# gvtulder/elasticdeform

Measured on AMD Instinct MI355X. Metric: Mvoxels/s fwd+grad, 256^3 fp32 order=3, higher is better.
Workload: dtype f32; 1 GPU; cfg2: 3D 256x256x256 float32, 5x5x5 grid sigma 5, order 3, mode mirror, prefilter on, deform_grid + deform_grid_gradient per step, one volume per GPU; parallelism=1 volume per GPU, no collective

## Files before the change

### elasticdeform_amd/csrc/deform_k1z.hip

```cpp
#include <hip/hip_runtime.h>

#include <cstring>
#include <type_traits>

#include "ed_device.h"
#include "ed_gridfilter.h"
#include "ed_params.h"
#include "ed_tile.h"
#include "ed_workspace.h"
#include "ed_zwalk.h"

namespace ed {
namespace tile {

#ifdef EDHIP_K1_STATS
__device__ unsigned long long g_k1z_stats[8];
#define ZSTAT(K, N) atomicAdd(&g_k1z_stats[K], (unsigned long long)(N))
#else
#define ZSTAT(K, N) do { } while (0)
#endif

namespace {


enum : int {
    kZAny = 1,
    kZStaged = 2,
    kZFast = 4,
    kZDma = 8,
    kZXin = 16,
    kZZYin = 32,
    kZUnfit = 64,
    kZGen = 128,
};
struct ZRecU {
    int b0z, b0y, b0x, flags, pitch, ez, ey, ex, goff, plane;
};
typedef int zv8i __attribute__((ext_vector_type(8)));
typedef const __attribute__((address_space(4))) zv8i* crec_p;
__device__ __forceinline__ ZRecU zrec_unpack(const zv8i& v)
{
    ZRecU r;
    r.b0z = v[0];
    r.b0y = v[1];
    r.b0x = v[2];
    r.flags = v[3];
    r.pitch = (v[3] >> 8) & 255;
    r.ez = v[4] & 1023;
    r.ey = (v[4] >> 10) & 1023;
    r.ex = (int)((unsigned)v[4] >> 20);
    r.goff = v[5];
    r.plane = r.ey * r.pitch;
    return r;
}
__device__ __forceinline__ ZRecU zrec_load(crec_p p)
{
    const zv8i v = *p;
    return zrec_unpack(v);
}

enum : int { kZHeavy = 0, kZFix = 1, kZLight = 2, kZCursor = 3 };
__host__ __device__ __forceinline__ int zctl(int parity, int word, int xcd) { return (parity * 4 + word) * 8 + xcd; }

__device__ __forceinline__ void zaxis_entry(const GridGeom& g, int a, int oi, double* w, int* idx)
{
    const double cp = control_coordinate(g.ncp[a], (int64_t)oi + g.off[a], g.in_len[a]);
    const int64_t start = window_start(cp, 3);
    const bool edge = start < 0 || start + 3 >= g.ncp[a];
    spline_weights(cp, 3, w);
#pragma unroll
    for (int l = 0; l < 4; ++l)
        idx[l] = edge ? mirror_i32((int)start + l, (int)g.ncp[a]) : (int)start + l;
}

constexpr int kGeoBlock = 256;
constexpr int kGeoWaves = kGeoBlock / 64;
__global__ __launch_bounds__(kGeoBlock) void k1z_geo_kernel(const GridGeom g, const HotGeom hg, const ZGeom zg,
                                                          const GridPrefilter gp)
{
    extern __shared__ __attribute__((aligned(16))) char smem[];
    const int tid = threadIdx.x;
    const int lane = tid & 63;
    const int wave = uni(tid >> 6);
    const int sample = blockIdx.y;
    const int ncpz = (int)g.ncp[0], ncpy = (int)g.ncp[1], ncpx = (int)g.ncp[2];
    const int nyx = ncpy * ncpx;
    const int ngrid = 3 * ncpz * nyx;
    double* sG = reinterpret_cast<double*>(smem);
    double* sR = sG + ngrid;
    AxTab* sAx = reinterpret_cast<AxTab*>(sR + 64 * ncpz * 3);
    double* sMax = reinterpret_cast<double*>(sAx + 16);
    AxTab* sZ = reinterpret_cast<AxTab*>(sMax + 3 * kGeoWaves);
    int* sCls = reinterpret_cast<int*>(sZ + 4 * hg.tiles[0]);
    int* sBox = sCls + hg.tiles[0];
    int* sCnt = sBox + 64 * hg.tiles[0];
    const int ty = blockIdx.x / hg.tiles[2], tx = blockIdx.x - ty * hg.tiles[2];
    if (ED_DBG(hg.dbg, 1 << 23))
        return;
#ifdef EDHIP_EXPERIMENTS
#define ZTICK(K) do { if (hg.dbgbuf && tid == 0) hg.dbgbuf[(size_t)(blockIdx.x + blockIdx.y * gridDim.x) * 16 + (K)] = __builtin_readcyclecounter(); } while (0)
#else
#define ZTICK(K) do { } while (0)
#endif
    ZTICK(0);

    if (gp.total > 0 && !ED_DBG(hg.dbg, 1 << 28)) {
        grid_prefilter_in_lds<kGeoBlock>(gp, sG, tid);
        if (blockIdx.x == 0 && sample == 0)
            for (int e = tid; e < gp.total; e += kGeoBlock)
                store_cast(gp.out + (int64_t)e * gp.elem_size, gp.dtype, sG[e]);
    } else {
        const char* disp = g.disp + (int64_t)sample * zg.disp_bstride;
        for (int e = tid; e < ngrid; e += kGeoBlock) {
            const int h = e / (ncpz * nyx), r = e - h * (ncpz * nyx);
            const int j0 = r / nyx, j = r - j0 * nyx;
            const int j1 = j / ncpx, j2 = j - j1 * ncpx;
            sG[e] = load_as_double(disp + g.disp_stride[0] * h + g.disp_stride[1] * j0 + g.disp_stride[2] * j1 +
                                       g.disp_stride[3] * j2, g.disp_dtype);
        }
        __syncthreads();
    }
    ZTICK(1);
    if (blockIdx.x == 0 && sample == 0 && tid == 0 && zg.hint) {
        if (zg.hint_host)
            __hip_atomic_store(zg.hint_host, ((unsigned long long)(unsigned)zg.hint[1] << 32) | (unsigned)zg.hint[0],
                               __ATOMIC_RELAXED, __HIP_MEMORY_SCOPE_SYSTEM);
        zg.hint[0] = 0;
        zg.hint[1] = (int)zg.hint_seq;
    }
    for (int h = 0; h < 3 && !ED_DBG(hg.dbg, 1 << 29); ++h) {
        double m = 0.0;
        for (int e = tid; e < ncpz * nyx; e += kGeoBlock)
            m = fmax(m, fabs(sG[h * ncpz * nyx + e]));
        for (int sh = 32; sh >= 1; sh >>= 1)
            m = fmax(m, __shfl_xor(m, sh));
        if (lane == 0)
            sMax[h * kGeoWaves + wave] = m;
    }
    ZTICK(2);
    if (tid < 16 && !ED_DBG(hg.dbg, 1 << 30)) {
        const int a = tid < 8 ? 1 : 2;
        const int oi = min((tid < 8 ? ty : tx) * kT + (tid & 7), hg.out_len[a] - 1);
        AxTab t;
        zaxis_entry(g, a, oi, t.w, t.idx);
        sAx[tid] = t;
    }
    for (int e = tid; e < 4 * hg.tiles[0] && !ED_DBG(hg.dbg, 1 << 26); e += kGeoBlock) {
        const int tz = e >> 2, nz = min(kT, hg.out_len[0] - tz * kT);
        AxTab t;
        zaxis_entry(g, 0, tz * kT + ((e & 3) * (nz - 1)) / 3, t.w, t.idx);
        sZ[e] = t;
    }
    if (blockIdx.x == 0 && sample == 0 && hg.nstep) {
        for (long long ss = tid; ss < hg.nsteps; ss += kGeoBlock) {
            long long vol_off = 0, img_off = 0, r = ss;
            for (int l = 0; l < hg.nstep; ++l) {
                const long long q = r / hg.step_len[l];
                const long long c = r - q * hg.step_len[l];
                vol_off += hg.vol_step[l] * c;
                img_off += hg.img_step[l] * c;
                r = q;
            }
            zg.steps[2 * ss] = vol_off;
            zg.steps[2 * ss + 1] = img_off;
        }
    }
    if (blockIdx.x == 0 && sample == 0 && tid == 0) {
        ZGen* zn = reinterpret_cast<ZGen*>(zg.zgen);
        for (int h = 0; h < 3; ++h) {
            zn->in_len[h] = hg.in_len[h];
            zn->out_len[h] = hg.out_len[h];
            zn->off[h] = hg.off[h];
            zn->period[h] = hg.period[h];
            zn->inv_period[h] = hg.inv_period[h];
            zn->offd[h] = (double)hg.off[h];
        }
        for (int k = 0; k < 12; ++k)
            zn->aff[k] = hg.affine[k];
        zn->mode = hg.mode;
        zn->cval = hg.cval;
        zn->hint = hg.hint;
    }
    if (blockIdx.x == 0 && sample == 0) {
        AxTab* zt = const_cast<AxTab*>(zg.zt);
        for (int oz = tid; oz < hg.out_len[0]; oz += kGeoBlock) {
            AxTab t;
            zaxis_entry(g, 0, oz, t.w, t.idx);
#pragma unroll
            for (int l = 0; l < 4; ++l)
                t.idx[l] *= 32;
            zt[oz] = t;
        }
    }
    __syncthreads();
    ZTICK(3);
    double slack[3];
#pragma unroll
    for (int h = 0; h < 3; ++h) {
        double m = 0.0;
        for (int w = 0; w < kGeoWaves; ++w)
            m = fmax(m, sMax[h * kGeoWaves + w]);
        const double sl = zg.slack_scale * m;
        slack[h] = sl >= 0.02 ? (sl <= 0.75 ? sl : 0.75) : 0.02;
    }
    ZTICK(4);
    if (!ED_DBG(hg.dbg, 1 << 25)) {
        const int col = tid & 63;
        const AxTab ay = sAx[col >> 3];
        const AxTab ax = sAx[8 + (col & 7)];
        int rowoff[4];
#pragma unroll
        for (int ly = 0; ly < 4; ++ly)
            rowoff[ly] = ay.idx[ly] * ncpx;
        for (int r = tid >> 6; r < ncpz * 3; r += kGeoWaves) {
            const int kz = r / 3, h = r - kz * 3;
            const double* gp0 = sG + (h * ncpz + kz) * nyx;
            double acc = 0.0;
#pragma unroll
            for (int ly = 0; ly < 4; ++ly) {
                const double* row = gp0 + rowoff[ly];
                double t = ax.w[0] * row[ax.idx[0]];
#pragma unroll
                for (int lx = 1; lx < 4; ++lx)
                    t = fma(ax.w[lx], row[ax.idx[lx]], t);
                acc = fma(ay.w[ly], t, acc);
            }
            sR[col * (ncpz * 3) + r] = acc;
        }
        __syncthreads();
        double* rg = const_cast<double*>(zg.r) + (int64_t)sample * zg.r_bstride;
        const int rowlen = 8 * 4 * ncpz;
        for (int e = tid; e < 8 * rowlen; e += kGeoBlock) {
            const int py = e / rowlen, j = e - py * rowlen;
            const int px = j / (4 * ncpz), jj = j - px * (4 * ncpz);
            const int kz = jj >> 2, h = jj & 3;
            const int oy = ty * kT + py, ox = tx * kT + px;
            if (oy < hg.out_len[1] && ox < hg.out_len[2])
                rg[((int64_t)oy * hg.out_len[2] + ox) * (4 * ncpz) + jj] = h < 3 ? sR[(py * 8 + px) * (ncpz * 3) + kz * 3 + h] : 0.0;
        }
    }
    __syncthreads();
    ZTICK(5);
    const int order = zg.order;
    const int H = order / 2, NT = order + 1, kPadX = NT & 1;
    const int ny = min(kT, hg.out_len[1] - ty * kT), nx = min(kT, hg.out_len[2] - tx * kT);
    const int py = (((lane >> 2) & 3) * (ny - 1)) / 3, px = ((lane & 3) * (nx - 1)) / 3;
    const double* rc = sR + (py * 8 + px) * (ncpz * 3);
    for (int tz = wave; tz < hg.tiles[0] && !ED_DBG(hg.dbg, 1 << 24); tz += kGeoWaves) {
        const int nz = min(kT, hg.out_len[0] - tz * kT);
        const int pz = ((lane >> 4) * (nz - 1)) / 3;
        const int o[3] = {tz * kT + pz, ty * kT + py, tx * kT + px};
        const AxTab& ze = sZ[tz * 4 + (lane >> 4)];
        double d[3];
#pragma unroll
        for (int h = 0; h < 3; ++h) {
            d[h] = ze.w[0] * rc[ze.idx[0] * 3 + h];
#pragma unroll
            for (int l = 1; l < 4; ++l)
                d[h] = fma(ze.w[l], rc[ze.idx[l] * 3 + h], d[h]);
        }
        double c[3];
        int lo[3], hi[3];
#pragma unroll
        for (int h = 0; h < 3; ++h) {
            if (hg.has_affine)
                c[h] = fma(hg.affine[h * 4 + 2], (double)o[2],
                           fma(hg.affine[h * 4 + 0], (double)o[0],
                               fma(hg.affine[h * 4 + 1], (double)o[1], hg.affine[h * 4 + 3] + (double)hg.off[h]))) + d[h];
            else
                c[h] = (double)(o[h] + hg.off[h]) + d[h];
            const double cr = (order & 1) ? c[h] : c[h] + 0.5;
            lo[h] = (int)floor(cr - slack[h]);
            hi[h] = (int)floor(cr + slack[h]);
        }
        bool out_of_fast = false;
#pragma unroll
        for (int h = 0; h < 3; ++h)
            out_of_fast = out_of_fast || lo[h] < ((order & 1) ? 0 : 1) || hi[h] > hg.in_len[h] - 2;
        const bool fast = nz == kT && ny == kT && nx == kT && !__any(out_of_fast);
        box_reduce<4>(lo, hi);
        int* dst = sBox + (tz * 8 + (lane >> 4)) * 8;
        if ((lane & 15) == 0) {
#pragma unroll
            for (int h = 0; h < 3; ++h) {
                dst[h] = lo[h];
                dst[4 + h] = hi[h];
            }
        }
        if (lane == 0)
            dst[3] = fast ? 1 : 0;
        if (!fast) {
            bool cst = false;
#pragma unroll
            for (int h = 0; h < 3; ++h) {
                double m = c[h];
                if (!(m >= 0.0 && m <= (double)(hg.in_len[h] - 1)))
                    m = map_coordinate_fast(m, hg.in_len[h], hg.mode, hg.period[h], hg.inv_period[h]);
                cst = cst || !(m > -1.0);
                const double mr = (order & 1) ? m : m + 0.5;
                lo[h] = (int)floor(mr - slack[h]);
                hi[h] = (int)floor(mr + slack[h]);
            }
            if (cst) {
#pragma unroll
                for (int h = 0; h < 3; ++h) {
                    lo[h] = 0x7fffffff;
                    hi[h] = (int)0x80000000;
                }
            }
            box_reduce<4>(lo, hi);
            if ((lane & 15) == 0) {
#pragma unroll
                for (int h = 0; h < 3; ++h) {
                    dst[32 + h] = lo[h];
                    dst[36 + h] = hi[h];
                }
            }
        }
    }
    __syncthreads();
    ZTICK(6);
    for (int tz = tid; tz < hg.tiles[0] && !ED_DBG(hg.dbg, 1 << 27); tz += kGeoBlock) {
        const int tile_id = sample * hg.ntiles + (tz * hg.tiles[1] + ty) * hg.tiles[2] + tx;
        int cls = 0;
        bool hint0 = false, slow0 = false, half_fit[2] = {false, false};
#pragma unroll 1
        for (int part = 0; part < 3; ++part) {
            const int* sb = sBox + tz * 64;
            const bool fast = sb[3] != 0;
            const int r0 = part == 2 ? 2 : 0, r1 = part == 1 ? 2 : 3;
            int blo[3], bhi[3];
            bool any = true;
#pragma unroll
            for (int h = 0; h < 3; ++h) {
                int rlo = 0x7fffffff, rhi = (int)0x80000000, lo = 0x7fffffff, hi = (int)0x80000000;
                for (int r = r0; r <= r1; ++r) {
                    rlo = min(rlo, sb[r * 8 + h]);
                    rhi = max(rhi, sb[r * 8 + 4 + h]);
                    lo = min(lo, sb[(fast ? 0 : 32) + r * 8 + h]);
                    hi = max(hi, sb[(fast ? 0 : 32) + r * 8 + 4 + h]);
                }
                if (!fast) {
                    any = any && hi >= lo;
                    const int lowfold = hg.mode == EDHIP_MODE_REFLECT ? -1 : 0;
                    if (rlo < ((order & 1) ? 0 : 1) && rhi >= lowfold)
                        lo = min(lo, lowfold);
                    if (rhi > hg.in_len[h] - 2 && rlo <= hg.in_len[h] - 1)
                        hi = max(hi, hg.in_len[h] - 1);
                }
                blo[h] = lo - H;
                bhi[h] = hi - H + order + (h == 2 ? kPadX : 0);
            }
            if (!any) {
                blo[0] = blo[1] = blo[2] = 0;
                bhi[0] = bhi[1] = bhi[2] = -1;
            }
            any = bhi[0] >= blo[0] && bhi[1] >= blo[1] && bhi[2] >= blo[2];
            unsigned ext[3];
#pragma unroll
            for (int h = 0; h < 3; ++h)
                ext[h] = (unsigned)bhi[h] - (unsigned)blo[h] + 1u;
            const int pitch = ext[2] <= 16u ? 16 : (ext[2] <= 24u ? 24 : (ext[2] <= 32u ? 32 : (ext[2] <= 48u ? 48 : 0)));
            const bool sane = any && ext[0] < 1024u && ext[1] < 1024u;
            const int nrows = sane ? (int)(ext[0] * ext[1]) : 0;
            const bool fits = sane && pitch > 0 && nrows * pitch <= hg.box_cap;
            const bool dma = fits && blo[2] >= 0 && blo[2] + pitch + 1 <= hg.in_len[2];
            const bool xin = fits && blo[2] >= 0 && blo[2] + (int)ext[2] <= hg.in_len[2];
            const bool zyin = fits && blo[0] >= 0 && blo[0] + (int)ext[0] <= hg.in_len[0] && blo[1] >= 0 &&
                              blo[1] + (int)ext[1] <= hg.in_len[1];
            const bool fastA = part == 0 && fast && fits && dma && zyin;
            const int flags = (any ? kZAny : 0) | (fits ? kZStaged : 0) | (fastA ? kZFast : kZGen) | (dma ? kZDma : 0) |
                              (xin ? kZXin : 0) | (zyin ? kZZYin : 0) | (any && !fits ? kZUnfit : 0);
            const int4 w0 = make_int4(blo[0], blo[1], blo[2], flags | (pitch << 8));
            const int4 w1 = make_int4(sane ? (int)(ext[0] | (ext[1] << 10) | (ext[2] << 20)) : 0,
                                      (dma && zyin) ? blo[0] * hg.vol_sz + blo[1] * hg.vol_sy + blo[2] : 0, 0, 0);
            if (part == 0) {
                hint0 = any && !(sane && pitch > 0 && nrows * pitch <= hg.small_cap);
                slow0 = fits && !dma;
                cls = (flags & kZUnfit) ? 3 : ((flags & kZFast) ? 1 : 2);
                int4* dst = reinterpret_cast<int4*>(zg.recs + (size_t)tile_id * 8);
                dst[0] = w0;
                dst[1] = w1;
                if (hg.boxes) {
                    int* bx = hg.boxes + (size_t)tile_id * 8;
#pragma unroll
                    for (int h = 0; h < 3; ++h) {
                        bx[h] = blo[h];
                        bx[3 + h] = bhi[h] - ((h == 2 && any) ? kPadX : 0);
                    }
                }
                if (cls != 3)
                    break;
            } else {
                half_fit[part - 1] = fits || !any;
                int4* dst = reinterpret_cast<int4*>(zg.recs_half + ((size_t)tile_id * 2 + (part - 1)) * 8);
                dst[0] = w0;
                dst[1] = w1;
            }
        }
        const bool split = cls == 3 && half_fit[0] && half_fit[1];
        ZSTAT(cls == 3 ? (split ? 6 : 5) : (cls == 1 ? 3 : 4), 1);
        sCls[tz] = cls | (split ? 4 : 0) | (hint0 ? 8 : 0) | ((cls == 2 && slow0) || split ? 16 : 0);
    }
    __syncthreads();
    ZTICK(7);
    {
        const int zstrips = (hg.tiles[0] + zg.strip_tiles - 1) / zg.strip_tiles;
        int* sCntL = reinterpret_cast<int*>(sMax);
        if (tid < 4)
            sCnt[tid] = 0;
        if (tid < 2)
            sCntL[tid] = 0;
        __syncthreads();
        int slotG = -1, slotL = -1, slotF = -1, sidv = 0;
        if (tid < zstrips) {
            int info = 0, ngen = 0;
            bool slow = false, f = false;
            for (int k = 0; k < zg.strip_tiles && tid * zg.strip_tiles + k < hg.tiles[0]; ++k) {
                const int c = sCls[tid * zg.strip_tiles + k];
                info |= (c & 15) << (4 * k);
                ngen += ((c & 3) == 2 || (c & 7) == 7) ? 1 : 0;
                slow = slow || (c & 16) != 0;
                f = f || (c & 7) == 3;
            }
            const size_t sid = (size_t)sample * zg.nstrips + ((size_t)tid * hg.tiles[1] + ty) * hg.tiles[2] + tx;
            sidv = (int)sid;
            zg.sinfo[sid] = info;
            zg.missed[sid] = f ? 2 : 0;
            if (ngen && (slow || ngen >= 3) && !ED_DBG(hg.dbg, 1 << 13))
                slotG = atomicAdd(&sCnt[0], 1);
            else if (ngen)
                slotL = atomicAdd(&sCntL[0], 1);
            if (f)
                slotF = atomicAdd(&sCnt[1], 1);
        }
        __syncthreads();
        const int xcd = (tx + ty + sample) & 7;
        if (tid == 0) {
            sCnt[2] = sCnt[0] ? atomicAdd(&zg.ctl[zctl(zg.parity, kZHeavy, xcd)], sCnt[0]) : 0;
            sCnt[3] = sCnt[1] ? atomicAdd(&zg.ctl[zctl(zg.parity, kZFix, xcd)], sCnt[1]) : 0;
            sCntL[1] = sCntL[0] ? atomicAdd(&zg.ctl[zctl(zg.parity, kZLight, xcd)], sCntL[0]) : 0;
        }
        if (blockIdx.x == 0 && sample == 0 && tid < 32)
            zg.ctl[zctl(1 - zg.parity, tid >> 3, tid & 7)] = 0;
        __syncthreads();
        if (slotG >= 0)
            zg.list_g[(size_t)(sCnt[2] + slotG) * 8 + xcd] = sidv;
        if (slotL >= 0)
            zg.list_g[(size_t)(zg.total_strips - 1 - (sCntL[1] + slotL)) * 8 + xcd] = sidv;
        if (slotF >= 0)
            zg.list_f[(size_t)(sCnt[3] + slotF) * 8 + xcd] = sidv;
    }
    ZTICK(8);
#undef ZTICK
}


struct ZVox {
    int addr[2];
    float frac[2][3];
    int flg;
};
struct ZStrip {
    int tz0, ty, tx, ntile, sample, id;
};
__device__ __forceinline__ bool k1z_strip(int total_strips, int nstrips, int tiles_z, int tiles_y, int tiles_x, int strip_tiles, int deal,
                                          ZStrip& sp, int b)
{
    const int x = b & 7, j = b >> 3;
    const int r = j / deal;
    int s = (r * 8 + ((x + r) & 7)) * deal + (j - r * deal);
    if (s >= total_strips)
        return false;
    sp.id = s;
    sp.sample = s / nstrips;
    s -= sp.sample * nstrips;
    sp.tx = s % tiles_x;
    s /= tiles_x;
    sp.ty = s % tiles_y;
    sp.tz0 = (s / tiles_y) * strip_tiles;
    sp.ntile = min(strip_tiles, tiles_z - sp.tz0);
    return true;
}
inline unsigned k1z_grid(int total_strips, int deal)
{
    const int chunks = (total_strips + deal - 1) / deal;
    return (unsigned)(((chunks + 7) / 8) * 8 * deal);
}

template <int ORDER, int PITCH>
__device__ __forceinline__ float k1z_gather(const float* bp, int plane, int pitch_rt, const float* w0, const float* w1, const float* w2)
{
    constexpr int NT = ORDER + 1;
    constexpr int NTX = NT + (NT & 1);
    float a0 = 0.f;
#pragma unroll
    for (int l0 = 0; l0 < NT; ++l0) {
        const float* pp = bp + l0 * plane;
        float a1 = 0.f;
#pragma unroll
        for (int l1 = 0; l1 < NT; ++l1) {
            const float* rp = pp + l1 * (PITCH ? PITCH : pitch_rt);
            float a2 = 0.f;
#pragma unroll
            for (int l2 = 0; l2 < NTX; l2 += 2) {
                const float2 pr = *reinterpret_cast<const float2*>(rp + l2);
                ED_NO_DS_MERGE();
                a2 = fmaf(w2[l2], pr.x, a2);
                a2 = fmaf(w2[l2 + 1], pr.y, a2);
            }
            a1 = fmaf(w1[l1], a2, a1);
        }
        a0 = fmaf(w0[l0], a1, a0);
    }
    return a0;
}
template <int ORDER>
__device__ __forceinline__ float k1z_voxel(const char* smem, int addr, const float (&frac)[3], int pitch, int plane)
{
    constexpr int NT = ORDER + 1;
    constexpr int NTX = NT + (NT & 1);
    float f0 = frac[0], f1 = frac[1], f2 = frac[2];
    asm volatile("" : "+v"(f0), "+v"(f1), "+v"(f2));
    float w0[NT], w1[NT], w2[NTX];
    weights_from_frac<float, ORDER>(f0, w0);
    weights_from_frac<float, ORDER>(f1, w1);
    weights_from_frac<float, ORDER>(f2, w2);
    if (NT & 1)
        w2[NT] = 0.f;
    const float* bp = reinterpret_cast<const float*>(smem + addr);
    return pitch == 16 ? k1z_gather<ORDER, 16>(bp, plane, 16, w0, w1, w2) : k1z_gather<ORDER, 0>(bp, plane, pitch, w0, w1, w2);
}

struct ZFast {
    const float* vol;
    float* img;
    const double* r;
    const AxTab* zt;
    const int* recs;
    const int* recs_half;
    int* missed;
    int* hint;
    const int* sinfo;
    const int* list_g;
    int* list_f;
    int* ctl;
    int parity;
    const long long* steps;
    long long vol_bstride, img_bstride, r_bstride;
    int vol_sy, vol_sz, img_sy, img_sz;
    int box_cap, tiles_y, tiles_x, tiles_z, strip_tiles, nstrips, total_strips, ntiles;
    int rcol_bytes, out_y, out_x;
    int kz0, ky0, kx0;
    int io16, nsteps, deal;
    int dbg;
    double aff[12];
#ifdef EDHIP_EXPERIMENTS
    unsigned long long* dbgbuf;
#endif
};
#ifdef EDHIP_EXPERIMENTS
constexpr size_t kZDbgBase = (size_t)1 << 16;
#endif

template <int ORDER, bool AFFINE, bool OUT16, bool STEPS>
__device__ __forceinline__ void k1z_fast_body(const ZFast& a, const int vblock)
{
    constexpr int NT = ORDER + 1;
    constexpr int kPadX = NT & 1;
    constexpr int NTX = NT + kPadX;
    extern __shared__ __attribute__((aligned(16))) char smem[];
    ZStrip sp;
    if (!k1z_strip(a.total_strips, a.nstrips, a.tiles_z, a.tiles_y, a.tiles_x, a.strip_tiles, a.deal, sp, vblock))
        return;
    const int tid = threadIdx.x;
    const int lane = tid & 63;
    const int wave = uni(tid >> 6);
    const int io16 = OUT16 ? a.io16 : 0;
    const int ntile = sp.ntile;
    const size_t tile_step = (size_t)a.tiles_y * a.tiles_x;
    crec_p rec0 = (crec_p)(const void*)a.recs + ((size_t)sp.sample * a.ntiles + ((size_t)sp.tz0 * a.tiles_y + sp.ty) * a.tiles_x + sp.tx);
    const int sinfo = ((cint_p)(const void*)a.sinfo)[sp.id];
    if (a.hint && tid == 0) {
        const int nh = __builtin_popcount((unsigned)sinfo & 0x88888888u);
        if (nh)
            atomicAdd(a.hint, nh);
    }
    auto next_fast = [&](int t) {
        for (++t; t < ntile; ++t)
            if (((sinfo >> (4 * t)) & 3) == 1)
                break;
        return t;
    };
    int ti = next_fast(-1);
    if (ti >= ntile)
        return;

    const int box_cap = a.box_cap;
    const int odd_shift = (box_cap - 1) * 4;
    float* box0 = reinterpret_cast<float*>(smem);
    float* box1 = box0 + box_cap;
    const int vol_sz = a.vol_sz, vol_sy = a.vol_sy, img_sz = a.img_sz;

    const int yy = lane >> 3, xx = lane & 7;
    const int oy = sp.ty * kT + yy, ox = sp.tx * kT + xx;
    const int obase = oy * a.img_sy + ox;
// ... 476 lines not shown
        const int sinfo = ((cint_p)(const void*)a.sinfo)[sp.id];
        const bool missed = (((cint_p)(const void*)a.missed)[sp.id] & 1) != 0;
        if (!STEPS && false)
            (void)steps;
        const int oy = sp.ty * kT + yy, ox = sp.tx * kT + xx;
        const int obase = oy * a.img_sy + ox;
        const float* __restrict__ vol = a.vol + sp.sample * a.vol_bstride;
        float* img = a.img + sp.sample * a.img_bstride;
        const char* rcol = reinterpret_cast<const char*>(a.r + sp.sample * a.r_bstride) +
                           ((size_t)min(oy, a.out_y - 1) * a.out_x + min(ox, a.out_x - 1)) * (size_t)a.rcol_bytes;
        double Pyx[3];
#pragma unroll
        for (int h = 0; h < 3; ++h)
            Pyx[h] = AFFINE ? fma(zn->aff[h * 4 + 2], (double)ox, fma(zn->aff[h * 4 + 1], (double)oy, zn->aff[h * 4 + 3] + zn->offd[h])) : 0.0;
        ZTaps tp;
        tp.key[0] = tp.key[1] = tp.key[2] = tp.key[3] = -1;
        {
            if (missed && lane == 0)
                ZSTAT(0, 1);
            for (int ti = (int)(blockIdx.y >> 1); ti < ntile; ti += ntile) {
                const int c4 = (sinfo >> (4 * ti)) & 7;
                const int cls = c4 & 3;
                const bool split = c4 == 7;
                const bool whole = cls == 3 && !split;
                if (!whole && !missed)
                    continue;
#pragma unroll 1
                for (int i = (int)(blockIdx.y & 1); i < 2; i += 2) {
                    const ZRecU rc = zrec_load(split ? rech0 + ((size_t)ti * tile_step * 2 + i) : rec0 + (size_t)ti * tile_step);
                    const int oz = (sp.tz0 + ti) * kT + wave + 4 * i;
                    if (oz >= zn->out_len[0])
                        continue;
                    double zw[4];
                    k1z_slice(zt, rcol, oz, tp, zw);
                    if (oy >= zn->out_len[1] || ox >= zn->out_len[2])
                        continue;
                    double d[3];
                    k1z_disp(tp, zw, d);
                    const int b[3] = {oz + zn->off[0], oy + zn->off[1], ox + zn->off[2]};
                    double P[3] = {0.0, 0.0, 0.0};
                    if (AFFINE) {
#pragma unroll
                        for (int h = 0; h < 3; ++h)
                            P[h] = fma(zn->aff[h * 4 + 0], (double)oz, Pyx[h]);
                    }
                    int st[3], raw[3];
                    float fr[3];
                    const bool cst = tile_coords<ORDER, AFFINE, float>(zn->in_len, &zn->mode, zn->period, zn->inv_period, d, b,
                                                                       P, st, fr, raw);
                    if (!whole) {
                        const bool gen = cls != 1;
                        if (gen && cst)
                            continue;
                        const int rz = (gen ? st[0] : raw[0]) - rc.b0z, ry = (gen ? st[1] : raw[1]) - rc.b0y,
                                  rx = (gen ? st[2] : raw[2]) - rc.b0x;
                        const bool inside = rz >= 0 && rz + NT <= rc.ez && ry >= 0 && ry + NT <= rc.ey && rx >= 0 &&
                                            rx + NT + kPadX <= rc.ex;
                        if (inside)
                            continue;
                    }
                    int tap[3][NT];
                    float w[3][NT];
#pragma unroll
                    for (int h = 0; h < 3; ++h) {
                        weights_from_frac<float, ORDER>(fr[h], w[h]);
                        const int stride = h == 0 ? vol_sz : (h == 1 ? vol_sy : 1);
#pragma unroll
                        for (int l = 0; l < NT; ++l)
                            tap[h][l] = mirror_i32(st[h] + l, zn->in_len[h]) * stride;
                    }
                    const long long ooff = (long long)oz * img_sz + obase;
                    ZSTAT(whole ? 2 : 1, 1);
                    for (int ss = 0; ss < nsteps; ++ss) {
                        float val = zn->cval;
                        if (!cst) {
                            const float* src = vol + (STEPS ? steps[2 * ss] : 0);
                            float a0 = 0.f;
#pragma unroll
                            for (int l0 = 0; l0 < NT; ++l0) {
                                float a1 = 0.f;
#pragma unroll
                                for (int l1 = 0; l1 < NT; ++l1) {
                                    const float* p1 = src + (tap[0][l0] + tap[1][l1]);
                                    float a2 = 0.f;
#pragma unroll
                                    for (int l2 = 0; l2 < NT; ++l2)
                                        a2 = fmaf(w[2][l2], p1[tap[2][l2]], a2);
                                    a1 = fmaf(w[1][l1], a2, a1);
                                }
                                a0 = fmaf(w[0][l0], a1, a0);
                            }
                            val = a0;
                        }
                        store_out<OUT16>(img, (STEPS ? steps[2 * ss + 1] : 0) + ooff, val, io16);
                    }
                }
            }
        }
    }
}

template <int ORDER, bool AFFINE, bool OUT16, bool STEPS>
hipError_t launch_k1z_kernels(const ZFast& zf, const void* znp, unsigned ngen, unsigned nfix, size_t lds, hipStream_t stream)
{
    const unsigned nfast = k1z_grid(zf.total_strips, zf.deal);
    const unsigned fast_rows = nfast >> 3, gen_rows = ngen >> 3;
    unsigned every = gen_rows ? fast_rows / gen_rows + 1 : 2;
    if (const char* ev = ed_env("EDHIP_ZEVERY"))
        every = (unsigned)atoi(ev);
    if (every < 2)
        every = 2;
    hipLaunchKernelGGL((k1z_tile_kernel<ORDER, AFFINE, OUT16, STEPS>), dim3(nfast + ngen), dim3(kBlock), lds, stream, zf, (czgen_p)znp,
                       (int)ngen, (int)every);
    hipError_t e = hipGetLastError();
    if (e != hipSuccess)
        return e;
    hipLaunchKernelGGL((k1z_fix_kernel<ORDER, AFFINE, OUT16, STEPS>), dim3(nfix, 2 * zf.strip_tiles), dim3(kBlock), 0, stream, zf, (czgen_p)znp);
    return hipGetLastError();
}
template <int ORDER, bool AFFINE, bool OUT16>
hipError_t launch_k1z_variant(const ZFast& zf, const void* zn, unsigned ngen, unsigned nfix, size_t lds, hipStream_t stream,
                              bool steps)
{
    return steps ? launch_k1z_kernels<ORDER, AFFINE, OUT16, true>(zf, zn, ngen, nfix, lds, stream)
                 : launch_k1z_kernels<ORDER, AFFINE, OUT16, false>(zf, zn, ngen, nfix, lds, stream);
}
template <int ORDER>
hipError_t launch_k1z_order(const HotGeom& hg, const ZFast& zf, const void* zn, unsigned ngen, unsigned nfix, size_t lds, hipStream_t stream)
{
    const bool steps = hg.nstep != 0;
    if (hg.io16)
        return hg.has_affine ? launch_k1z_variant<ORDER, true, true>(zf, zn, ngen, nfix, lds, stream, steps)
                             : launch_k1z_variant<ORDER, false, true>(zf, zn, ngen, nfix, lds, stream, steps);
    return hg.has_affine ? launch_k1z_variant<ORDER, true, false>(zf, zn, ngen, nfix, lds, stream, steps)
                         : launch_k1z_variant<ORDER, false, false>(zf, zn, ngen, nfix, lds, stream, steps);
}

}

size_t k1z_lds_bytes(int* box_cap, bool large)
{
    size_t budget = large ? 52 * 1024 : 31 * 1024;
    if (const char* kb = ed_env("EDHIP_ZKB"))
        budget = (size_t)atoi(kb) * 1024;
    size_t cap = budget / 8;
    cap = ((cap - 56) / 64) * 64 + 56;
    *box_cap = (int)cap;
    return 2 * 4 * cap + 16;
}

size_t k1z_geo_lds_bytes(const GridGeom& g, const HotGeom& hg)
{
    const size_t ngrid = 3 * (size_t)g.ncp[0] * (size_t)g.ncp[1] * (size_t)g.ncp[2];
    return 8 * ngrid + 8 * 64 * 3 * (size_t)g.ncp[0] + 16 * sizeof(AxTab) + 3 * kGeoWaves * 8 + (sizeof(AxTab) * 4 + 4 + 256) * (size_t)hg.tiles[0] + 16;
}

size_t k1z_r_bytes(const GridGeom& g) { return 8 * (size_t)g.out_len[1] * (size_t)g.out_len[2] * 4 * (size_t)g.ncp[0]; }

bool k1z_supported(const GridGeom& g)
{
    const size_t ngrid = 3 * (size_t)g.ncp[0] * (size_t)g.ncp[1] * (size_t)g.ncp[2];
    const size_t tiles_z = (size_t)((g.out_len[0] + kT - 1) / kT);
    return ngrid <= 4096 && g.ncp[0] <= 16 &&
           8 * ngrid + 8 * 64 * 3 * (size_t)g.ncp[0] + 16 * sizeof(AxTab) + 3 * kGeoWaves * 8 + (sizeof(AxTab) * 4 + 4 + 256) * tiles_z + 16 <= 60 * 1024;
}

hipError_t launch_k1z_geo(const GridGeom& g, const HotGeom& hg, const ZGeom& zg, const GridPrefilter& gp, int nbatch,
                          hipStream_t stream)
{
    hipLaunchKernelGGL(k1z_geo_kernel, dim3((unsigned)(hg.tiles[1] * hg.tiles[2]), (unsigned)nbatch), dim3(kGeoBlock),
                       k1z_geo_lds_bytes(g, hg), stream, g, hg, zg, gp);
    if (ed_env("EDHIP_GEO_TWICE"))
        hipLaunchKernelGGL(k1z_geo_kernel, dim3((unsigned)(hg.tiles[1] * hg.tiles[2]), (unsigned)nbatch), dim3(kGeoBlock),
                           k1z_geo_lds_bytes(g, hg), stream, g, hg, zg, gp);
    return hipGetLastError();
}

hipError_t launch_k1z(const HotGeom& hg, const ZGeom& zg, int order, size_t lds, hipStream_t stream)
{
    ZFast zf;
    memset(&zf, 0, sizeof(zf));
    zf.vol = hg.vol_r;
    zf.img = hg.img_w;
    zf.r = zg.r;
    zf.zt = zg.zt;
    zf.recs = zg.recs;
    zf.recs_half = zg.recs_half;
    zf.missed = zg.missed;
    zf.hint = hg.hint;
    zf.sinfo = zg.sinfo;
    zf.list_g = zg.list_g;
    zf.list_f = zg.list_f;
    zf.ctl = zg.ctl;
    zf.parity = zg.parity;
    zf.steps = zg.steps;
    zf.vol_bstride = hg.vol_bstride;
    zf.img_bstride = hg.img_bstride;
    zf.r_bstride = zg.r_bstride;
    zf.vol_sy = hg.vol_sy;
    zf.vol_sz = hg.vol_sz;
    zf.img_sy = hg.img_sy;
    zf.img_sz = hg.img_sz;
    zf.box_cap = hg.box_cap;
    zf.tiles_z = hg.tiles[0];
    zf.tiles_y = hg.tiles[1];
    zf.tiles_x = hg.tiles[2];
    zf.strip_tiles = zg.strip_tiles;
    zf.nstrips = zg.nstrips;
    zf.total_strips = zg.total_strips;
    zf.ntiles = hg.ntiles;
    zf.rcol_bytes = 32 * zg.ncpz;
    zf.out_y = hg.out_len[1];
    zf.out_x = hg.out_len[2];
    const int H = order / 2;
    zf.kz0 = (hg.has_affine ? 0 : hg.off[0]) - H;
    zf.ky0 = (hg.has_affine ? 0 : hg.off[1]) - H;
    zf.kx0 = (hg.has_affine ? 0 : hg.off[2]) - H;
    zf.io16 = hg.io16;
    zf.nsteps = (int)hg.nsteps;
    zf.dbg = hg.dbg;
#ifdef EDHIP_EXPERIMENTS
    zf.dbgbuf = hg.dbgbuf;
#endif
    zf.deal = 4 * hg.tiles[2];
    while (zf.deal > 1 && zg.total_strips < 16 * zf.deal)
        zf.deal >>= 1;
    if (const char* dl = ed_env("EDHIP_ZDEAL"))
        zf.deal = atoi(dl) >= 1 ? atoi(dl) : zf.deal;
    for (int h = 0; h < 3; ++h) {
        for (int k = 0; k < 3; ++k)
            zf.aff[h * 4 + k] = hg.affine[h * 4 + k];
        zf.aff[h * 4 + 3] = hg.affine[h * 4 + 3] + (double)hg.off[h];
    }
    const void* zn = zg.zgen;
    unsigned ngen = (unsigned)(zg.total_strips < 1280 ? ((zg.total_strips + 7) / 8) * 8 : 1280);
    if (const char* ng = ed_env("EDHIP_ZNGEN"))
        ngen = (unsigned)((atoi(ng) + 7) / 8 * 8);
    const unsigned nfix = (unsigned)(zg.total_strips < 512 ? ((zg.total_strips + 7) / 8) * 8 : 512);
    switch (order) {
    case 1: return launch_k1z_order<1>(hg, zf, zn, ngen, nfix, lds, stream);
    case 2: return launch_k1z_order<2>(hg, zf, zn, ngen, nfix, lds, stream);
    case 3: return launch_k1z_order<3>(hg, zf, zn, ngen, nfix, lds, stream);
    default: return hipErrorNotSupported;
    }
}

#ifdef EDHIP_K1_STATS
extern "C" int edhip_debug_k1z_stats(unsigned long long* out8)
{
    unsigned long long z[8] = {0, 0, 0, 0, 0, 0, 0, 0};
    if (hipMemcpyFromSymbol(out8, HIP_SYMBOL(g_k1z_stats), sizeof(z)) != hipSuccess)
        return 1;
    return hipMemcpyToSymbol(HIP_SYMBOL(g_k1z_stats), z, sizeof(z)) != hipSuccess;
}
#endif

}
}
```

### elasticdeform_amd/csrc/ed_gridfilter.h

```cpp
#pragma once
#include "ed_device.h"
#include "ed_params.h"

namespace ed {

template <int N>
__device__ __forceinline__ void grid_filter_line(double* c, int inner, double z, double gain, double zn1)
{
#pragma clang fp contract(off)
    double v[N];
#pragma unroll
    for (int i = 0; i < N; ++i)
        v[i] = c[i * inner] * gain;
    double c0 = v[0] + zn1 * v[N - 1];
    double zi = z;
#pragma unroll
    for (int i = 1; i < N - 1; ++i) {
        c0 += zi * (v[i] + zn1 * v[N - 1 - i]);
        zi *= z;
    }
    c0 /= 1 - zn1 * zn1;
    v[0] = c0;
#pragma unroll
    for (int i = 1; i < N; ++i)
        v[i] += z * v[i - 1];
    v[N - 1] = (z * v[N - 2] + v[N - 1]) * z / (z * z - 1);
#pragma unroll
    for (int i = N - 2; i >= 0; --i)
        v[i] = z * (v[i + 1] - v[i]);
#pragma unroll
    for (int i = 0; i < N; ++i)
        c[i * inner] = v[i];
}

template <int NT>
__device__ __forceinline__ void grid_prefilter_in_lds(const GridPrefilter& p, double* s, int tid)
{
#pragma clang fp contract(off)
    const int total = p.total;
    for (int e = tid; e < total; e += NT) {
        int r = e;
        int64_t off = 0;
        for (int d = p.ndim - 1; d >= 0; --d) {
            const int q = r / p.shape[d];
            off += (int64_t)(r - q * p.shape[d]) * p.stride_bytes[d];
            r = q;
        }
        s[e] = load_as_double(p.in + off, p.dtype);
    }
    __syncthreads();
    const double z = p.pole, gain = p.gain;
    for (int ax = 1; ax < p.ndim; ++ax) {
        const int n = p.shape[ax];
        int inner = 1;
        for (int d = ax + 1; d < p.ndim; ++d)
            inner *= p.shape[d];
        const int nlines = total / n;
        if (n >= 2) {
            const double zn1 = p.pole_pow[ax];
            for (int line = tid; line < nlines; line += NT) {
                const int outer = line / inner, in = line - outer * inner;
                double* c = s + (int64_t)outer * n * inner + in;
                switch (n) {
                case 2: grid_filter_line<2>(c, inner, z, gain, zn1); continue;
                case 3: grid_filter_line<3>(c, inner, z, gain, zn1); continue;
                case 4: grid_filter_line<4>(c, inner, z, gain, zn1); continue;
                case 5: grid_filter_line<5>(c, inner, z, gain, zn1); continue;
                case 6: grid_filter_line<6>(c, inner, z, gain, zn1); continue;
                case 7: grid_filter_line<7>(c, inner, z, gain, zn1); continue;
                case 8: grid_filter_line<8>(c, inner, z, gain, zn1); continue;
                default: break;
                }
                for (int i = 0; i < n; ++i)
                    c[i * inner] *= gain;
                double c0 = c[0] + zn1 * c[(n - 1) * inner];
                double zi = z;
                for (int i = 1; i < n - 1; ++i) {
                    c0 += zi * (c[i * inner] + zn1 * c[(n - 1 - i) * inner]);
                    zi *= z;
                }
                c0 /= 1 - zn1 * zn1;
                c[0] = c0;
                for (int i = 1; i < n; ++i)
                    c[i * inner] += z * c[(i - 1) * inner];
                c[(n - 1) * inner] = (z * c[(n - 2) * inner] + c[(n - 1) * inner]) * z / (z * z - 1);
                for (int i = n - 2; i >= 0; --i)
                    c[i * inner] = z * (c[(i + 1) * inner] - c[i * inner]);
            }
        }
        __syncthreads();
        if (p.dtype != EDHIP_F64) {
            for (int e = tid; e < total; e += NT) {
                char tmp[8];
                store_cast(tmp, p.dtype, s[e]);
                s[e] = load_as_double(tmp, p.dtype);
            }
            __syncthreads();
        }
    }
}

}
```

Measured before the change: 26530 Mvoxels/s.

## Overlap geometry side work with grid prefilter and cut barriers in k1z_geo_kernel

```diff
diff --git a/elasticdeform_amd/csrc/deform_k1z.hip b/elasticdeform_amd/csrc/deform_k1z.hip
--- a/elasticdeform_amd/csrc/deform_k1z.hip
+++ b/elasticdeform_amd/csrc/deform_k1z.hip
@@ -75,6 +75,7 @@
 
 constexpr int kGeoBlock = 256;
 constexpr int kGeoWaves = kGeoBlock / 64;
+constexpr int kGeoBoxInts = 65;
 __global__ __launch_bounds__(kGeoBlock) void k1z_geo_kernel(const GridGeom g, const HotGeom hg, const ZGeom zg,
                                                           const GridPrefilter gp)
 {
@@ -93,7 +94,7 @@
     AxTab* sZ = reinterpret_cast<AxTab*>(sMax + 3 * kGeoWaves);
     int* sCls = reinterpret_cast<int*>(sZ + 4 * hg.tiles[0]);
     int* sBox = sCls + hg.tiles[0];
-    int* sCnt = sBox + 64 * hg.tiles[0];
+    int* sCnt = sBox + kGeoBoxInts * hg.tiles[0];
     const int ty = blockIdx.x / hg.tiles[2], tx = blockIdx.x - ty * hg.tiles[2];
     if (ED_DBG(hg.dbg, 1 << 23))
         return;
@@ -102,86 +103,65 @@
 #else
 #define ZTICK(K) do { } while (0)
 #endif
-    ZTICK(0);
-
-    if (gp.total > 0 && !ED_DBG(hg.dbg, 1 << 28)) {
-        grid_prefilter_in_lds<kGeoBlock>(gp, sG, tid);
-        if (blockIdx.x == 0 && sample == 0)
-            for (int e = tid; e < gp.total; e += kGeoBlock)
-                store_cast(gp.out + (int64_t)e * gp.elem_size, gp.dtype, sG[e]);
-    } else {
-        const char* disp = g.disp + (int64_t)sample * zg.disp_bstride;
-        for (int e = tid; e < ngrid; e += kGeoBlock) {
-            const int h = e / (ncpz * nyx), r = e - h * (ncpz * nyx);
-            const int j0 = r / nyx, j = r - j0 * nyx;
-            const int j1 = j / ncpx, j2 = j - j1 * ncpx;
-            sG[e] = load_as_double(disp + g.disp_stride[0] * h + g.disp_stride[1] * j0 + g.disp_stride[2] * j1 +
-                                       g.disp_stride[3] * j2, g.disp_dtype);
-        }
-        __syncthreads();
-    }
-    ZTICK(1);
-    if (blockIdx.x == 0 && sample == 0 && tid == 0 && zg.hint) {
-        if (zg.hint_host)
-            __hip_atomic_store(zg.hint_host, ((unsigned long long)(unsigned)zg.hint[1] << 32) | (unsigned)zg.hint[0],
-                               __ATOMIC_RELAXED, __HIP_MEMORY_SCOPE_SYSTEM);
-        zg.hint[0] = 0;
-        zg.hint[1] = (int)zg.hint_seq;
-    }
-    for (int h = 0; h < 3 && !ED_DBG(hg.dbg, 1 << 29); ++h) {
-        double m = 0.0;
-        for (int e = tid; e < ncpz * nyx; e += kGeoBlock)
-            m = fmax(m, fabs(sG[h * ncpz * nyx + e]));
-        for (int sh = 32; sh >= 1; sh >>= 1)
-            m = fmax(m, __shfl_xor(m, sh));
-        if (lane == 0)
-            sMax[h * kGeoWaves + wave] = m;
-    }
-    ZTICK(2);
-    if (tid < 16 && !ED_DBG(hg.dbg, 1 << 30)) {
-        const int a = tid < 8 ? 1 : 2;
-        const int oi = min((tid < 8 ? ty : tx) * kT + (tid & 7), hg.out_len[a] - 1);
-        AxTab t;
-        zaxis_entry(g, a, oi, t.w, t.idx);
-        sAx[tid] = t;
-    }
-    for (int e = tid; e < 4 * hg.tiles[0] && !ED_DBG(hg.dbg, 1 << 26); e += kGeoBlock) {
-        const int tz = e >> 2, nz = min(kT, hg.out_len[0] - tz * kT);
-        AxTab t;
-        zaxis_entry(g, 0, tz * kT + ((e & 3) * (nz - 1)) / 3, t.w, t.idx);
-        sZ[e] = t;
-    }
-    if (blockIdx.x == 0 && sample == 0 && hg.nstep) {
-        for (long long ss = tid; ss < hg.nsteps; ss += kGeoBlock) {
-            long long vol_off = 0, img_off = 0, r = ss;
-            for (int l = 0; l < hg.nstep; ++l) {
-                const long long q = r / hg.step_len[l];
-                const long long c = r - q * hg.step_len[l];
-                vol_off += hg.vol_step[l] * c;
-                img_off += hg.img_step[l] * c;
-                r = q;
-            }
-            zg.steps[2 * ss] = vol_off;
-            zg.steps[2 * ss + 1] = img_off;
-        }
-    }
-    if (blockIdx.x == 0 && sample == 0 && tid == 0) {
-        ZGen* zn = reinterpret_cast<ZGen*>(zg.zgen);
-        for (int h = 0; h < 3; ++h) {
-            zn->in_len[h] = hg.in_len[h];
-            zn->out_len[h] = hg.out_len[h];
-            zn->off[h] = hg.off[h];
-            zn->period[h] = hg.period[h];
-            zn->inv_period[h] = hg.inv_period[h];
-            zn->offd[h] = (double)hg.off[h];
-        }
-        for (int k = 0; k < 12; ++k)
-            zn->aff[k] = hg.affine[k];
-        zn->mode = hg.mode;
-        zn->cval = hg.cval;
-        zn->hint = hg.hint;
-    }
-    if (blockIdx.x == 0 && sample == 0) {
+#ifdef EDHIP_EXPERIMENTS
+    if (hg.dbgbuf && tid == 0)
+        hg.dbgbuf[(size_t)(blockIdx.x + blockIdx.y * gridDim.x) * 16] =
+            (__builtin_readcyclecounter() & ((1ull << 44) - 1)) | ((unsigned long long)(__builtin_amdgcn_s_getreg(63492) & 0xffff) << 44) |
+            ((unsigned long long)(__builtin_amdgcn_s_getreg(63508) & 15) << 60);
+#endif
+
+    const auto side_work = [&]() {
+        const int nent = 16 + 4 * hg.tiles[0];
+        for (int q = kGeoBlock - 1 - tid; q < nent; q += kGeoBlock) {
+            const bool zs = q >= 16;
+            if (ED_DBG(hg.dbg, zs ? 1 << 26 : 1 << 30))
+                continue;
+            const int e = q - 16, tz = e >> 2, nz = min(kT, hg.out_len[0] - tz * kT);
+            const int a = zs ? 0 : (q < 8 ? 1 : 2);
+            const int oi = zs ? tz * kT + ((e & 3) * (nz - 1)) / 3 : min((q < 8 ? ty : tx) * kT + (q & 7), hg.out_len[a] - 1);
+            AxTab t;
+            zaxis_entry(g, a, oi, t.w, t.idx);
+            (zs ? sZ + e : sAx + q)[0] = t;
+        }
+        if (blockIdx.x != 0 || sample != 0)
+            return;
+        if (tid == 0 && zg.hint) {
+            if (zg.hint_host)
+                __hip_atomic_store(zg.hint_host, ((unsigned long long)(unsigned)zg.hint[1] << 32) | (unsigned)zg.hint[0],
+                                   __ATOMIC_RELAXED, __HIP_MEMORY_SCOPE_SYSTEM);
+            zg.hint[0] = 0;
+            zg.hint[1] = (int)zg.hint_seq;
+        }
+        if (hg.nstep) {
+            for (long long ss = tid; ss < hg.nsteps; ss += kGeoBlock) {
+                long long vol_off = 0, img_off = 0, r = ss;
+                for (int l = 0; l < hg.nstep; ++l) {
+                    const long long q = r / hg.step_len[l];
+                    const long long c = r - q * hg.step_len[l];
+                    vol_off += hg.vol_step[l] * c;
+                    img_off += hg.img_step[l] * c;
+                    r = q;
+                }
+                zg.steps[2 * ss] = vol_off;
+                zg.steps[2 * ss + 1] = img_off;
+            }
+        }
+        if (tid == 0) {
+            ZGen* zn = reinterpret_cast<ZGen*>(zg.zgen);
+            for (int h = 0; h < 3; ++h) {
+                zn->in_len[h] = hg.in_len[h];
+                zn->out_len[h] = hg.out_len[h];
+                zn->off[h] = hg.off[h];
+                zn->period[h] = hg.period[h];
+                zn->inv_period[h] = hg.inv_period[h];
+                zn->offd[h] = (double)hg.off[h];
+            }
+            for (int k = 0; k < 12; ++k)
+                zn->aff[k] = hg.affine[k];
+            zn->mode = hg.mode;
+            zn->cval = hg.cval;
+            zn->hint = hg.hint;
+        }
         AxTab* zt = const_cast<AxTab*>(zg.zt);
         for (int oz = tid; oz < hg.out_len[0]; oz += kGeoBlock) {
             AxTab t;
@@ -191,16 +171,47 @@
                 t.idx[l] *= 32;
             zt[oz] = t;
         }
-    }
-    __syncthreads();
+    };
+    unsigned long long* sMaxBits = reinterpret_cast<unsigned long long*>(sMax);
+    const auto slack_max = [&](int h, double v) {
+        const double a = fabs(v);
+        if (a == a && !ED_DBG(hg.dbg, 1 << 29))
+            atomicMax(sMaxBits + h * 4 + (lane & 3), (unsigned long long)__double_as_longlong(a));
+    };
+    if (tid < 12)
+        sMaxBits[tid] = 0;
+    lds_barrier();
+
+    if (gp.total > 0 && !ED_DBG(hg.dbg, 1 << 28)) {
+        grid_prefilter_in_lds<kGeoBlock>(gp, sG, tid, side_work);
+        ZTICK(1);
+        const bool keep = blockIdx.x == 0 && sample == 0;
+        const int comp = ncpz * nyx;
+        for (int e = tid; e < ngrid; e += kGeoBlock) {
+            const double v = sG[e];
+            slack_max((e >= comp ? 1 : 0) + (e >= 2 * comp ? 1 : 0), v);
+            if (keep)
+                store_cast(gp.out + (int64_t)e * gp.elem_size, gp.dtype, v);
+        }
+    } else {
+        side_work();
+        const char* disp = g.disp + (int64_t)sample * zg.disp_bstride;
+        GridCounter4 c(tid, kGeoBlock, ncpz, ncpy, ncpx);
+        for (int e = tid; e < ngrid; e += kGeoBlock, c.next()) {
+            const double v = load_as_double(disp + g.disp_stride[0] * c.i[0] + g.disp_stride[1] * c.i[1] + g.disp_stride[2] * c.i[2] +
+                                                g.disp_stride[3] * c.i[3], g.disp_dtype);
+            sG[e] = v;
+            slack_max(c.i[0], v);
+        }
+        ZTICK(1);
+    }
+    ZTICK(2);
+    lds_barrier();
     ZTICK(3);
     double slack[3];
 #pragma unroll
     for (int h = 0; h < 3; ++h) {
-        double m = 0.0;
-        for (int w = 0; w < kGeoWaves; ++w)
-            m = fmax(m, sMax[h * kGeoWaves + w]);
-        const double sl = zg.slack_scale * m;
+        const double sl = zg.slack_scale * fmax(fmax(sMax[h * 4], sMax[h * 4 + 1]), fmax(sMax[h * 4 + 2], sMax[h * 4 + 3]));
         slack[h] = sl >= 0.02 ? (sl <= 0.75 ? sl : 0.75) : 0.02;
     }
     ZTICK(4);
@@ -227,25 +238,33 @@
             }
             sR[col * (ncpz * 3) + r] = acc;
         }
-        __syncthreads();
+        lds_barrier();
+        ZTICK(5);
         double* rg = const_cast<double*>(zg.r) + (int64_t)sample * zg.r_bstride;
-        const int rowlen = 8 * 4 * ncpz;
-        for (int e = tid; e < 8 * rowlen; e += kGeoBlock) {
-            const int py = e / rowlen, j = e - py * rowlen;
-            const int px = j / (4 * ncpz), jj = j - px * (4 * ncpz);
-            const int kz = jj >> 2, h = jj & 3;
-            const int oy = ty * kT + py, ox = tx * kT + px;
-            if (oy < hg.out_len[1] && ox < hg.out_len[2])
-                rg[((int64_t)oy * hg.out_len[2] + ox) * (4 * ncpz) + jj] = h < 3 ? sR[(py * 8 + px) * (ncpz * 3) + kz * 3 + h] : 0.0;
-        }
-    }
-    __syncthreads();
-    ZTICK(5);
+        const int prow = tid >> 5, oy = ty * kT + prow;
+        const int npair = min(kT, hg.out_len[2] - tx * kT) * 2 * ncpz;
+        if (oy < hg.out_len[1]) {
+            double2* dst = reinterpret_cast<double2*>(rg + ((int64_t)oy * hg.out_len[2] + tx * kT) * (4 * ncpz));
+            const double* src = sR + prow * 8 * (ncpz * 3);
+            for (int j = tid & 31; j < npair; j += 32) {
+                const double* v = src + 3 * (j >> 1) + 2 * (j & 1);
+                dst[j] = make_double2(v[0], (j & 1) ? 0.0 : v[1]);
+            }
+        }
+        ZTICK(6);
+    }
+    ZTICK(7);
     const int order = zg.order;
     const int H = order / 2, NT = order + 1, kPadX = NT & 1;
     const int ny = min(kT, hg.out_len[1] - ty * kT), nx = min(kT, hg.out_len[2] - tx * kT);
     const int py = (((lane >> 2) & 3) * (ny - 1)) / 3, px = ((lane & 3) * (nx - 1)) / 3;
     const double* rc = sR + (py * 8 + px) * (ncpz * 3);
+    double am[12];
+#pragma unroll
+    for (int k = 0; k < 12; ++k)
+        am[k] = hg.has_affine ? hg.affine[k] : ((k & 3) == (k >> 2) ? 1.0 : 0.0);
+    const double half = (order & 1) ? 0.0 : 0.5;
+    ZTICK(8);
     for (int tz = wave; tz < hg.tiles[0] && !ED_DBG(hg.dbg, 1 << 24); tz += kGeoWaves) {
         const int nz = min(kT, hg.out_len[0] - tz * kT);
         const int pz = ((lane >> 4) * (nz - 1)) / 3;
@@ -263,13 +282,9 @@
         int lo[3], hi[3];
 #pragma unroll
         for (int h = 0; h < 3; ++h) {
-            if (hg.has_affine)
-                c[h] = fma(hg.affine[h * 4 + 2], (double)o[2],
-                           fma(hg.affine[h * 4 + 0], (double)o[0],
-                               fma(hg.affine[h * 4 + 1], (double)o[1], hg.affine[h * 4 + 3] + (double)hg.off[h]))) + d[h];
-            else
-                c[h] = (double)(o[h] + hg.off[h]) + d[h];
-            const double cr = (order & 1) ? c[h] : c[h] + 0.5;
+            c[h] = fma(am[h * 4 + 2], (double)o[2],
+                       fma(am[h * 4 + 0], (double)o[0], fma(am[h * 4 + 1], (double)o[1], am[h * 4 + 3] + (double)hg.off[h]))) + d[h];
+            const double cr = c[h] + half;
             lo[h] = (int)floor(cr - slack[h]);
             hi[h] = (int)floor(cr + slack[h]);
         }
@@ -279,7 +294,7 @@
             out_of_fast = out_of_fast || lo[h] < ((order & 1) ? 0 : 1) || hi[h] > hg.in_len[h] - 2;
         const bool fast = nz == kT && ny == kT && nx == kT && !__any(out_of_fast);
         box_reduce<4>(lo, hi);
-        int* dst = sBox + (tz * 8 + (lane >> 4)) * 8;
+        int* dst = sBox + tz * kGeoBoxInts + (lane >> 4) * 8;
         if ((lane & 15) == 0) {
 #pragma unroll
             for (int h = 0; h < 3; ++h) {
@@ -297,7 +312,7 @@
                 if (!(m >= 0.0 && m <= (double)(hg.in_len[h] - 1)))
                     m = map_coordinate_fast(m, hg.in_len[h], hg.mode, hg.period[h], hg.inv_period[h]);
                 cst = cst || !(m > -1.0);
-                const double mr = (order & 1) ? m : m + 0.5;
+                const double mr = m + half;
                 lo[h] = (int)floor(mr - slack[h]);
                 hi[h] = (int)floor(mr + slack[h]);
             }
@@ -318,15 +333,16 @@
             }
         }
     }
-    __syncthreads();
-    ZTICK(6);
+    ZTICK(9);
+    lds_barrier();
+    ZTICK(10);
     for (int tz = tid; tz < hg.tiles[0] && !ED_DBG(hg.dbg, 1 << 27); tz += kGeoBlock) {
         const int tile_id = sample * hg.ntiles + (tz * hg.tiles[1] + ty) * hg.tiles[2] + tx;
         int cls = 0;
         bool hint0 = false, slow0 = false, half_fit[2] = {false, false};
 #pragma unroll 1
         for (int part = 0; part < 3; ++part) {
-            const int* sb = sBox + tz * 64;
+            const int* sb = sBox + tz * kGeoBoxInts;
             const bool fast = sb[3] != 0;
             const int r0 = part == 2 ? 2 : 0, r1 = part == 1 ? 2 : 3;
             int blo[3], bhi[3];
@@ -334,11 +350,15 @@
 #pragma unroll
             for (int h = 0; h < 3; ++h) {
                 int rlo = 0x7fffffff, rhi = (int)0x80000000, lo = 0x7fffffff, hi = (int)0x80000000;
-                for (int r = r0; r <= r1; ++r) {
-                    rlo = min(rlo, sb[r * 8 + h]);
-                    rhi = max(rhi, sb[r * 8 + 4 + h]);
-                    lo = min(lo, sb[(fast ? 0 : 32) + r * 8 + h]);
-                    hi = max(hi, sb[(fast ? 0 : 32) + r * 8 + 4 + h]);
+#pragma unroll
+                for (int r = 0; r < 4; ++r) {
+                    const bool in = r >= r0 && r <= r1;
+                    const int a = sb[r * 8 + h], b = sb[r * 8 + 4 + h];
+                    const int ma = sb[(fast ? 0 : 32) + r * 8 + h], mb = sb[(fast ? 0 : 32) + r * 8 + 4 + h];
+                    rlo = in ? min(rlo, a) : rlo;
+                    rhi = in ? max(rhi, b) : rhi;
+                    lo = in ? min(lo, ma) : lo;
+                    hi = in ? max(hi, mb) : hi;
                 }
                 if (!fast) {
                     any = any && hi >= lo;
@@ -402,16 +422,16 @@
         ZSTAT(cls == 3 ? (split ? 6 : 5) : (cls == 1 ? 3 : 4), 1);
         sCls[tz] = cls | (split ? 4 : 0) | (hint0 ? 8 : 0) | ((cls == 2 && slow0) || split ? 16 : 0);
     }
-    __syncthreads();
-    ZTICK(7);
+    int* sCntL = reinterpret_cast<int*>(sMax);
+    if (tid >= kGeoBlock - 4)
+        sCnt[tid - (kGeoBlock - 4)] = 0;
+    if (tid >= kGeoBlock - 2)
+        sCntL[tid - (kGeoBlock - 2)] = 0;
+    ZTICK(11);
+    lds_barrier();
+    ZTICK(12);
     {
         const int zstrips = (hg.tiles[0] + zg.strip_tiles - 1) / zg.strip_tiles;
-        int* sCntL = reinterpret_cast<int*>(sMax);
-        if (tid < 4)
-            sCnt[tid] = 0;
-        if (tid < 2)
-            sCntL[tid] = 0;
-        __syncthreads();
         int slotG = -1, slotL = -1, slotF = -1, sidv = 0;
         if (tid < zstrips) {
             int info = 0, ngen = 0;
@@ -434,7 +454,8 @@
             if (f)
                 slotF = atomicAdd(&sCnt[1], 1);
         }
-        __syncthreads();
+        lds_barrier();
+        ZTICK(13);
         const int xcd = (tx + ty + sample) & 7;
         if (tid == 0) {
             sCnt[2] = sCnt[0] ? atomicAdd(&zg.ctl[zctl(zg.parity, kZHeavy, xcd)], sCnt[0]) : 0;
@@ -443,7 +464,8 @@
         }
         if (blockIdx.x == 0 && sample == 0 && tid < 32)
             zg.ctl[zctl(1 - zg.parity, tid >> 3, tid & 7)] = 0;
-        __syncthreads();
+        lds_barrier();
+        ZTICK(14);
         if (slotG >= 0)
             zg.list_g[(size_t)(sCnt[2] + slotG) * 8 + xcd] = sidv;
         if (slotL >= 0)
@@ -451,7 +473,7 @@
         if (slotF >= 0)
             zg.list_f[(size_t)(sCnt[3] + slotF) * 8 + xcd] = sidv;
     }
-    ZTICK(8);
+    ZTICK(15);
 #undef ZTICK
 }
 
@@ -1234,7 +1256,7 @@
 size_t k1z_geo_lds_bytes(const GridGeom& g, const HotGeom& hg)
 {
     const size_t ngrid = 3 * (size_t)g.ncp[0] * (size_t)g.ncp[1] * (size_t)g.ncp[2];
-    return 8 * ngrid + 8 * 64 * 3 * (size_t)g.ncp[0] + 16 * sizeof(AxTab) + 3 * kGeoWaves * 8 + (sizeof(AxTab) * 4 + 4 + 256) * (size_t)hg.tiles[0] + 16;
+    return 8 * ngrid + 8 * 64 * 3 * (size_t)g.ncp[0] + 16 * sizeof(AxTab) + 3 * kGeoWaves * 8 + (sizeof(AxTab) * 4 + 4 + 4 * kGeoBoxInts) * (size_t)hg.tiles[0] + 16;
 }
 
 size_t k1z_r_bytes(const GridGeom& g) { return 8 * (size_t)g.out_len[1] * (size_t)g.out_len[2] * 4 * (size_t)g.ncp[0]; }
diff --git a/elasticdeform_amd/csrc/ed_gridfilter.h b/elasticdeform_amd/csrc/ed_gridfilter.h
--- a/elasticdeform_amd/csrc/ed_gridfilter.h
+++ b/elasticdeform_amd/csrc/ed_gridfilter.h
@@ -33,22 +33,66 @@
         c[i * inner] = v[i];
 }
 
-template <int NT>
-__device__ __forceinline__ void grid_prefilter_in_lds(const GridPrefilter& p, double* s, int tid)
+struct GridCounter4 {
+    int i[4], n[4], d[4];
+    __device__ __forceinline__ GridCounter4(int e0, int step, int n1, int n2, int n3)
+    {
+        n[0] = 0;
+        n[1] = n1;
+        n[2] = n2;
+        n[3] = n3;
+#pragma unroll
+        for (int k = 3; k >= 1; --k) {
+            const int q = e0 / n[k], qs = step / n[k];
+            i[k] = e0 - q * n[k];
+            d[k] = step - qs * n[k];
+            e0 = q;
+            step = qs;
+        }
+        i[0] = e0;
+        d[0] = step;
+    }
+    __device__ __forceinline__ void next()
+    {
+        int carry = 0;
+#pragma unroll
+        for (int k = 3; k >= 1; --k) {
+            i[k] += d[k] + carry;
+            carry = i[k] >= n[k] ? 1 : 0;
+            i[k] -= carry ? n[k] : 0;
+        }
+        i[0] += d[0] + carry;
+    }
+};
+
+struct GridNoSideWork {
+    __device__ __forceinline__ void operator()() const {}
+};
+
+template <int NT, class Side = GridNoSideWork>
+__device__ __forceinline__ void grid_prefilter_in_lds(const GridPrefilter& p, double* s, int tid, Side side = Side())
 {
 #pragma clang fp contract(off)
     const int total = p.total;
-    for (int e = tid; e < total; e += NT) {
-        int r = e;
-        int64_t off = 0;
-        for (int d = p.ndim - 1; d >= 0; --d) {
-            const int q = r / p.shape[d];
-            off += (int64_t)(r - q * p.shape[d]) * p.stride_bytes[d];
-            r = q;
+    if (p.ndim == 4) {
+        GridCounter4 c(tid, NT, p.shape[1], p.shape[2], p.shape[3]);
+        for (int e = tid; e < total; e += NT, c.next())
+            s[e] = load_as_double(p.in + (c.i[0] * p.stride_bytes[0] + c.i[1] * p.stride_bytes[1] + c.i[2] * p.stride_bytes[2] +
+                                          c.i[3] * p.stride_bytes[3]), p.dtype);
+    } else {
+        for (int e = tid; e < total; e += NT) {
+            int r = e;
+            int64_t off = 0;
+            for (int d = p.ndim - 1; d >= 0; --d) {
+                const int q = r / p.shape[d];
+                off += (int64_t)(r - q * p.shape[d]) * p.stride_bytes[d];
+                r = q;
+            }
+            s[e] = load_as_double(p.in + off, p.dtype);
         }
-        s[e] = load_as_double(p.in + off, p.dtype);
     }
     __syncthreads();
+    side();
     const double z = p.pole, gain = p.gain;
     for (int ax = 1; ax < p.ndim; ++ax) {
         const int n = p.shape[ax];
```

Measured after the change: 26680 Mvoxels/s, median of 6. No clear change (+0.6%).
